# ChanghyeonKim93/nonlinear_optimizer_for_slam

Hardware: AMD Instinct MI355X
Metric: ndt6_gauss_newton_residual_blocks_per_sec (higher is better)
Workload: dtype f64

## Files before the change

nonlinear_optimizer_for_slam_amd/csrc/assemble_one_launch.hpp:

```cpp
#pragma once

#include "assemble_pass.hpp"

namespace nos {

constexpr size_t kSingleBlockMaxElements = size_t(1024) * 15;

template <typename Problem, typename T, int BLOCK, bool NT>
__device__ __forceinline__ int single_block_loop(const TiledLayout& L, typename Problem::Params& P, uint32_t n_chunks,
                                                 LmDevice& s_lm, double* s_sum, double* __restrict__ cost_history,
                                                 int history_capacity) {
  constexpr int kF = Problem::kFields;
  constexpr int kOut = Problem::kOut;
  const T* __restrict__ base = static_cast<const T*>(L.base);
  int executed = 0;
  while (s_lm.st.done == 0) {
    set_pose(P, &s_lm);
    T acc[kOut];
#pragma unroll
    for (int k = 0; k < kOut; ++k) acc[k] = T(0);
    constexpr uint32_t kRound = (kF * sizeof(T) > 64) ? 2 : 4;
    for (uint32_t c = 0; c < n_chunks; c += kRound) {
      T x[kRound][kF][1];
      uint64_t i0[kRound];
// ... 73 lines not shown
      asm volatile("s_waitcnt vmcnt(0)" ::: "memory");
      __hip_atomic_store(seq_host, seq, __ATOMIC_RELAXED, __HIP_MEMORY_SCOPE_SYSTEM);
    }
  }
}

constexpr uint32_t kClusterMaxBlocks = 256;
constexpr unsigned long long kClusterTimeoutTicks = 5000000ull;
constexpr unsigned long long kClusterMailboxTimeoutTicks = kMailboxTimeoutTicks;

struct ClusterCtl {
  unsigned int abort;
  unsigned int pad0[31];
  struct alignas(128) Arrival {
    unsigned int count;
    unsigned int pad[31];
  } arrival[8];
};

__device__ __forceinline__ double sc1_load(const double* p) {
  return __hip_atomic_load(p, __ATOMIC_RELAXED, __HIP_MEMORY_SCOPE_AGENT);
}
__device__ __forceinline__ void sc1_store(double* p, double v) {
  __hip_atomic_store(p, v, __ATOMIC_RELAXED, __HIP_MEMORY_SCOPE_AGENT);
}

__device__ __forceinline__ void state_store_sc1(LmDevice* lm, const nos_host::LmState& st) {
  double* d = reinterpret_cast<double*>(&lm->st);
  const double* s = reinterpret_cast<const double*>(&st);
  constexpr int kWords = int(sizeof(nos_host::LmState) / sizeof(double));
  static_assert(sizeof(nos_host::LmState) % sizeof(double) == 0, "LmState must be a whole number of doubles");
#pragma unroll
  for (int k = 0; k < kWords; ++k) sc1_store(d + k, s[k]);
}
__device__ __forceinline__ void state_load_sc1(const LmDevice* lm, nos_host::LmState& st) {
  const double* d = reinterpret_cast<const double*>(&lm->st);
  double* s = reinterpret_cast<double*>(&st);
  constexpr int kWords = int(sizeof(nos_host::LmState) / sizeof(double));
#pragma unroll
  for (int k = 0; k < kWords; ++k) s[k] = sc1_load(d + k);
}

template <int FIELDS, int ELEM>
struct ResidentShape;
template <>
struct ResidentShape<15, 8> { static constexpr int RI = 3, LI = 3; };
template <>
struct ResidentShape<15, 4> { static constexpr int RI = 3, LI = 4; };
template <>
struct ResidentShape<5, 8> { static constexpr int RI = 9, LI = 7; };
template <>
struct ResidentShape<5, 4> { static constexpr int RI = 10, LI = 14; };

template <typename Problem, typename T, int BLOCK, int RI, int LI, int SI = 0, bool SPF = false, bool NT = false>
__global__ __launch_bounds__(BLOCK) void solve_cluster_kernel(TiledLayout L, typename Problem::Params P,
                                                             double* __restrict__ partials, LmDevice* lm, ClusterCtl* ctl,
                                                             double* __restrict__ cost_history, int history_capacity,
                                                             double* entry_host, unsigned long long* seq_host,
                                                             unsigned long long seq, uint32_t items_per_lane,
                                                             const Mailbox* mail = nullptr, uint32_t stream_lds = 0u) {
  constexpr int kF = Problem::kFields;
  constexpr int kOut = Problem::kOut;
  constexpr int kCols = 32;
  constexpr int kSlices = BLOCK / kCols;
  const T* __restrict__ base = static_cast<const T*>(L.base);
  constexpr int kRF = kF;
  extern __shared__ __align__(16) unsigned char resident_raw[];
  T* resident = reinterpret_cast<T*>(resident_raw);
  __shared__ int s_flag;
  __shared__ int s_fast;
  __shared__ double red[kSlices][kCols];
  __shared__ double s_tot[kLmTotDoubles(kOut)];
  __shared__ double s_lmd_raw[(sizeof(LmDevice) + 7) / 8];
  LmDevice& s_lmd = *reinterpret_cast<LmDevice*>(s_lmd_raw);
  nos_host::LmState& s_state = s_lmd.st;
  [[maybe_unused]] __shared__ double s_local[kCols];
  [[maybe_unused]] __shared__ unsigned long long s_round0;
  const bool multi = mail != nullptr;

  const uint32_t J = items_per_lane & 0x7fffffffu;
  [[maybe_unused]] const bool allow_fast = (items_per_lane >> 31) == 0u;
  [[maybe_unused]] constexpr int kXccCol = 28;
  [[maybe_unused]] const unsigned int my_xcc = xcc_id();
  const uint64_t block_base = uint64_t(blockIdx.x) * BLOCK * J;
  auto fetch = [&](uint32_t j, T (&dst)[kRF]) -> bool {
    const uint64_t i = block_base + uint64_t(j) * BLOCK + threadIdx.x;
    const bool ok = i < L.n;
    const uint64_t ic = ok ? i : 0;
    const uint64_t off = (ic >> L.tile_shift) * L.tile_stride + (ic & L.tile_mask);
    T xt[kF][1];
#pragma unroll
    for (int f = 0; f < kF; ++f) load_items<T, 1, false>(base + field_offset<Problem>(L, ic, off, f), xt[f]);
#pragma unroll
    for (int f = 0; f < kF; ++f) dst[f] = ok ? xt[f][0] : T(0);
    return ok;
  };
  auto evaluate_resident = [&](const T (&xi)[kRF], bool ok, T (&acc_)[kOut]) { Problem::item(xi, P, ok, acc_); };
  T x[RI > 0 ? RI : 1][kRF];
  bool valid[RI > 0 ? RI : 1];
  static_assert(SI == 0 || (RI == 0 && LI == 0), "the streaming form keeps nothing resident");
  constexpr int kSI = SI > 0 ? SI : 1;
  [[maybe_unused]] T xs[kF][kSI];
  [[maybe_unused]] uint64_t xs_i0 = 0;
  [[maybe_unused]] const uint32_t my_rounds = blockIdx.x < J ? (J - blockIdx.x + gridDim.x - 1) / gridDim.x : 0u;
  [[maybe_unused]] const uint32_t lds_k = SI > 0 ? min(stream_lds, my_rounds > 0u ? my_rounds - 1u : 0u) : 0u;
  [[maybe_unused]] const uint32_t lds_r0 = lds_k > 0u ? my_rounds / (lds_k + 1u) : ~0u;
  [[maybe_unused]] const uint32_t lds_r1 = lds_k > 1u ? uint32_t(2ull * my_rounds / (lds_k + 1u)) : ~0u;
  [[maybe_unused]] const uint32_t lds_r2 = lds_k > 2u ? uint32_t(3ull * my_rounds / (lds_k + 1u)) : ~0u;
  [[maybe_unused]] auto lds_round = [&](uint32_t s) -> uint32_t { return s == 0u ? lds_r0 : s == 1u ? lds_r1 : s == 2u ? lds_r2 : ~0u; };
  [[maybe_unused]] auto fetch_chunk = [&](uint32_t c, T (&dst)[kF][kSI]) -> uint64_t {
    const uint64_t i0 = uint64_t(c) * (uint64_t(BLOCK) * kSI) + uint64_t(threadIdx.x) * kSI;
    const uint64_t off = (i0 >> L.tile_shift) * L.tile_stride + (i0 & L.tile_mask);
#pragma unroll
    for (int f = 0; f < kF; ++f) load_items<T, kSI, NT>(base + field_offset<Problem>(L, i0, off, f), dst[f]);
    return i0;
  };
  if constexpr (SI > 0) {
    if (blockIdx.x < J) xs_i0 = fetch_chunk(blockIdx.x, xs);
  }
#pragma unroll
  for (int j = 0; j < RI; ++j) {
    valid[j] = false;
    if (uint32_t(j) < J) {
      valid[j] = fetch(uint32_t(j), x[j]);
    } else {
#pragma unroll
      for (int f = 0; f < kRF; ++f) x[j][f] = T(0);
    }
  }
  if constexpr (LI > 0) {
    for (uint32_t j = RI; j < J; ++j) {
      T xi[kRF];
      (void)fetch(j, xi);
#pragma unroll
      for (int f = 0; f < kRF; ++f) resident[(size_t(j - RI) * kRF + f) * BLOCK + threadIdx.x] = xi[f];
    }
  }
  NOS_PROBE(if (threadIdx.x < 4) s_step_cycles[threadIdx.x] = 0ull;)
  if (threadIdx.x == 0) {
    s_lmd.settings = lm->settings;
    s_state = lm->st;
    s_flag = s_state.done != 0 ? 1 : 0;
    s_fast = 0;
    if (__hip_atomic_load(&ctl->abort, __ATOMIC_RELAXED, __HIP_MEMORY_SCOPE_AGENT) != 0u) s_flag = 2;
    if (multi && blockIdx.x == 0) s_round0 = *mail->round;
  }
  __syncthreads();
  [[maybe_unused]] const unsigned int group = blockIdx.x & 7u;
  const unsigned int n_groups = gridDim.x < 8u ? gridDim.x : 8u;
  unsigned int it = 0;
  int executed = 0;
  NOS_PROBE(unsigned long long tq[6] = {0, 0, 0, 0, 0, 0}, tp = 0;)
#define NOS_RES_STAMP(slot_) NOS_PROBE({ const unsigned long long now_ = wall_clock64(); tq[slot_] += now_ - tp; tp = now_; })
  while (s_flag == 0) {
    NOS_PROBE(tp = wall_clock64();)
    if constexpr (kOut == 28) {
#pragma unroll
      for (int k = 0; k < 9; ++k) P.R[k] = T(uniform_load(&s_state.R[k]));
#pragma unroll
      for (int k = 0; k < 3; ++k) P.t[k] = T(uniform_load(&s_state.t[k]));
    } else {
#pragma unroll
      for (int k = 0; k < 4; ++k) P.R2[k] = T(uniform_load(&s_state.R[k]));
#pragma unroll
      for (int k = 0; k < 2; ++k) P.t2[k] = T(uniform_load(&s_state.t[k]));
    }
    T acc[kOut];
#pragma unroll
    for (int k = 0; k < kOut; ++k) acc[k] = T(0);
    if constexpr (SI > 0) {
      const uint32_t n_chunks = J;
      auto evaluate = [&](const T (&xc)[kF][SI > 0 ? SI : 1], uint64_t i0) {
#pragma unroll
        for (int it = 0; it < (SI > 0 ? SI : 1); ++it) {
          T xi[kF];
#pragma unroll
          for (int f = 0; f < kF; ++f) xi[f] = xc[f][it];
          Problem::item(xi, P, (i0 + it) < L.n, acc);
        }
      };
      if constexpr (SPF) {
        for (uint32_t c = blockIdx.x; c < n_chunks; c += gridDim.x) {
          T xb[kF][SI > 0 ? SI : 1];
          uint64_t i1 = 0;
          const uint32_t cn = c + gridDim.x;
          if (cn < n_chunks) i1 = fetch_chunk(cn, xb);
          evaluate(xs, xs_i0);
#pragma unroll
          for (int f = 0; f < kF; ++f)
#pragma unroll
            for (int it = 0; it < (SI > 0 ? SI : 1); ++it) xs[f][it] = xb[f][it];
          xs_i0 = i1;
        }
      } else {
        auto lds_at = [&](uint32_t s, int f, int e) -> T& {
          return resident[((size_t(s) * kF + f) * BLOCK + threadIdx.x) * kSI + e];
        };
        auto evaluate_lds = [&](uint32_t s, uint32_t cl) {
          const uint64_t i0 = uint64_t(cl) * (uint64_t(BLOCK) * kSI) + uint64_t(threadIdx.x) * kSI;
#pragma unroll
          for (int e = 0; e < kSI; ++e) {
            T xi[kF];
#pragma unroll
            for (int f = 0; f < kF; ++f) xi[f] = lds_at(s, f, e);
            Problem::item(xi, P, (i0 + e) < L.n, acc);
          }
        };
        const bool from_lds = it != 0u;
        uint32_t s = 0;
        uint32_t next_res = lds_round(0u);
        auto evaluate_lds_rounds = [&](uint32_t k0, uint32_t k1) {
          for (uint32_t kr = k0; kr < k1; ++kr) {
            evaluate_lds(s, blockIdx.x + kr * gridDim.x);
            next_res = lds_round(++s);
          }
        };
        for (uint32_t k = 0; k < my_rounds;) {
          __builtin_amdgcn_sched_barrier(0);
          if (!from_lds && k == next_res) {
#pragma unroll
            for (int f = 0; f < kF; ++f)
#pragma unroll
              for (int e = 0; e < kSI; ++e) lds_at(s, f, e) = xs[f][e];
            next_res = lds_round(++s);
          }
          evaluate(xs, xs_i0);
          uint32_t kn = k + 1u;
          if (from_lds)
            for (uint32_t sn = s; kn == lds_round(sn); ++sn) ++kn;
          xs_i0 = fetch_chunk(blockIdx.x + (kn < my_rounds ? kn : 0u) * gridDim.x, xs);
          evaluate_lds_rounds(k + 1u, kn);
          k = kn;
        }
      }
      if constexpr (SPF) {
        if (blockIdx.x < n_chunks) xs_i0 = fetch_chunk(blockIdx.x, xs);
      }
    } else
    if (sizeof(T) == 8 && J >= uint32_t(RI)) {
#pragma unroll
      for (int j = 0; j < RI; ++j) evaluate_resident(x[j], valid[j], acc);
    } else {
#pragma unroll
      for (int j = 0; j < RI; ++j)
        if (uint32_t(j) < J) evaluate_resident(x[j], valid[j], acc);
    }
    if constexpr (LI > 0) {
      for (uint32_t j = RI; j < J; ++j) {
        T xi[kRF];
#pragma unroll
        for (int f = 0; f < kRF; ++f) xi[f] = resident[(size_t(j - RI) * kRF + f) * BLOCK + threadIdx.x];
        evaluate_resident(xi, (block_base + uint64_t(j) * BLOCK + threadIdx.x) < L.n, acc);
      }
    }
    double dacc[kOut];
#pragma unroll
    for (int k = 0; k < kOut; ++k) dacc[k] = double(acc[k]);
    NOS_RES_STAMP(0)
    {
      TaggedUnit* const block_units = reinterpret_cast<TaggedUnit*>(partials);
      TaggedUnit* const group_units = block_units + size_t(kClusterMaxBlocks) * 32;
      const unsigned long long tag = (seq << 24) | ((unsigned long long)it + 1ull);
      const double mine = block_reduce_value<kOut, BLOCK>(dacc);
      const bool probe = it == 0u && allow_fast;
      if (threadIdx.x < kOut) {
        if (s_fast != 0)
          tagged_store_plain(block_units + size_t(blockIdx.x) * 32 + threadIdx.x, mine, tag);
        else
          tagged_store(block_units + size_t(blockIdx.x) * 32 + threadIdx.x, mine, tag);
      } else if (probe && threadIdx.x == kXccCol) {
        tagged_store(block_units + size_t(blockIdx.x) * 32 + kXccCol, double(my_xcc), tag);
      }
      NOS_RES_STAMP(1)
      const unsigned long long deadline = wall_clock64() + (multi ? kClusterMailboxTimeoutTicks : kClusterTimeoutTicks);
      auto await = [&](const TaggedUnit* u, double* value) -> bool {
        unsigned int polls = 0;
        for (;;) {
          const TaggedUnit got = tagged_load(u);
          if (got.seq == tag) {
            *value = got.value;
            return true;
          }
          if ((++polls & 63u) == 0u &&
              (__hip_atomic_load(&ctl->abort, __ATOMIC_RELAXED, __HIP_MEMORY_SCOPE_AGENT) != 0u || wall_clock64() > deadline)) {
            __hip_atomic_store(&ctl->abort, 1u, __ATOMIC_RELAXED, __HIP_MEMORY_SCOPE_AGENT);
// ... 204 lines not shown
```

nonlinear_optimizer_for_slam_amd/csrc/nos_core.hip:

```cpp
#include "nos_internal.hpp"
#if defined(__x86_64__) && !defined(__HIP_DEVICE_COMPILE__)
#include <emmintrin.h>
#endif

#include <cxxabi.h>

namespace nosd {

namespace {
thread_local std::string g_last_error;
}

int fail(int status, const char* fmt, ...) {
  char buf[512];
  va_list ap;
  va_start(ap, fmt);
  vsnprintf(buf, sizeof buf, fmt, ap);
  va_end(ap);
  g_last_error = buf;
  return status;
}

const char* last_error_text() { return g_last_error.c_str(); }
void clear_last_error() { g_last_error.clear(); }
// ... 142 lines not shown
  constexpr bool kReproj = Problem::kFields == 5;
  if constexpr (sizeof(T) == 8) {
    if (variant == 0 && kReproj) variant = 7;
    switch (variant) {
      NOS_CASE(0, 1, 512, 3, 1)
      NOS_CASE(1, 1, 256, 3, 2)
      NOS_CASE(3, 2, 256, 2, 2)
      NOS_CASE_PP(7, 1, 512, kReproj ? 3 : 2, 1)
#ifdef NOS_ALL_VARIANTS
      NOS_CASE(2, 1, 256, 2, 2)
      NOS_CASE(4, 2, 512, 2, 1)
      NOS_CASE_PP(8, 2, 512, 2, 1)
#endif
    }
  } else {
    if (variant == 0) variant = kReproj ? 11 : 1;
    switch (variant) {
      NOS_CASE(1, 2, 512, 2, 1)
      NOS_CASE_PP(11, 2, 512, 2, 1)
#ifdef NOS_ALL_VARIANTS
      NOS_CASE(2, 1, 256, 4, 2)
      NOS_CASE(3, 2, 256, 5, 2)
      NOS_CASE(4, 2, 256, 4, 2)
      NOS_CASE(5, 1, 1024, 4, 1)
      NOS_CASE(6, 2, 1024, 4, 1)
      NOS_CASE(9, 2, 256, 3, 3)
      NOS_CASE_PP(12, 4, 512, 2, 1)
      NOS_CASE(13, 4, 256, 2, 1)
#endif
    }
  }
#undef NOS_CASE
#undef NOS_CASE_PP
  return fail(NOS_ERR_UNSUPPORTED, "launch geometry %d is not compiled into this build for this element type "
              "(default build: fp64 0, 1, 3, 7; fp32 1, 11; `make ALL_VARIANTS=1` builds the rest)", variant);
}

size_t resident_items_per_lane(int n_fields, int dtype) {
  if (n_fields == 15)
    return dtype == NOS_F64 ? size_t(nos::ResidentShape<15, 8>::RI + nos::ResidentShape<15, 8>::LI)
                            : size_t(nos::ResidentShape<15, 4>::RI + nos::ResidentShape<15, 4>::LI);
  if (n_fields == 5)
    return dtype == NOS_F64 ? size_t(nos::ResidentShape<5, 8>::RI + nos::ResidentShape<5, 8>::LI)
                            : size_t(nos::ResidentShape<5, 4>::RI + nos::ResidentShape<5, 4>::LI);
  return 1;
}

struct SingleBlockArgs {
  int cluster_blocks = 0;
  int items_per_lane = 1;
  int stream_chunks = 0;
  bool nt = false;
  int stream_lds_chunks = 0;
  bool stage1_sc1 = false;
  const nos::Mailbox* mail = nullptr;
  double* partials = nullptr;
  nos::ClusterCtl* ctl = nullptr;
  nos::LmDevice* lm;
  double* history;
  int history_capacity;
  double* entry;
  unsigned long long* seq_host;
  unsigned long long seq;
};

template <typename Problem, typename T>
int launch_single(const nos::TiledLayout& L, const typename Problem::Params& P, const SingleBlockArgs& a, hipStream_t stream) {
  constexpr int kBlock = 512;
  if (L.n_padded % kBlock != 0) return fail(NOS_ERR_INVALID_ARGUMENT, "n_padded %% 512 != 0");
  if (a.cluster_blocks > 0 && a.stream_chunks > 0) {
    constexpr int kSI = sizeof(T) == 8 ? 1 : 2;
    constexpr bool kSPF = false;
    constexpr size_t kChunk = size_t(kBlock) * kSI;
    if (L.n_padded % kChunk != 0 || (L.tile_stride != 0 && ((size_t(L.tile_mask) + 1) % kChunk) != 0))
      return fail(NOS_ERR_INVALID_ARGUMENT, "streaming solve: layout not a multiple of the %zu-item chunk", kChunk);
    if (size_t(a.stream_chunks) * kChunk != L.n_padded) return fail(NOS_ERR_INVALID_ARGUMENT, "streaming solve: chunk count does not match the layout");
    const auto kernel = a.nt ? nos::solve_cluster_kernel<Problem, T, kBlock, 0, 0, kSI, kSPF, true>
                             : nos::solve_cluster_kernel<Problem, T, kBlock, 0, 0, kSI, kSPF, false>;
    uint32_t lds = uint32_t(std::min(std::max(a.stream_lds_chunks, 0), 3));
    size_t dyn_bytes = lds * size_t(Problem::kFields) * kChunk * sizeof(T);
    if (dyn_bytes > size_t(48) * 1024 &&
        hipFuncSetAttribute(reinterpret_cast<const void*>(kernel), hipFuncAttributeMaxDynamicSharedMemorySize,
                            int(dyn_bytes)) != hipSuccess) {
      (void)hipGetLastError();
      lds = 0;
      dyn_bytes = 0;
    }
    t_last_kernel = reinterpret_cast<const void*>(kernel);
    hipLaunchKernelGGL(kernel, dim3(a.cluster_blocks), dim3(kBlock), dyn_bytes, stream, L, P, a.partials, a.lm, a.ctl, a.history,
                       a.history_capacity, a.entry, a.seq_host, a.seq, uint32_t(a.stream_chunks) | (a.stage1_sc1 ? 0x80000000u : 0u),
                       a.mail, lds);
    hipError_t e = hipGetLastError();
    if (e != hipSuccess) return fail(NOS_ERR_HIP, "streaming solve launch failed: %s", hipGetErrorString(e));
    return NOS_OK;
  }
  if (a.cluster_blocks > 0) {
    using Shape = nos::ResidentShape<Problem::kPlanes, int(sizeof(T))>;
    if (a.items_per_lane < 1 || a.items_per_lane > Shape::RI + Shape::LI)
      return fail(NOS_ERR_INVALID_ARGUMENT, "resident solve: %d items per lane do not fit (%d + %d)", a.items_per_lane,
                  Shape::RI, Shape::LI);
    const auto kernel = nos::solve_cluster_kernel<Problem, T, kBlock, Shape::RI, Shape::LI>;
    const size_t lds_items = a.items_per_lane > Shape::RI ? size_t(a.items_per_lane - Shape::RI) : 0;
    const size_t dyn_bytes = lds_items * size_t(Problem::kFields) * kBlock * sizeof(T);
    if (dyn_bytes > size_t(48) * 1024) {
      const hipError_t ea = hipFuncSetAttribute(reinterpret_cast<const void*>(kernel),
                                                hipFuncAttributeMaxDynamicSharedMemorySize, int(dyn_bytes));
      if (ea != hipSuccess) return fail(NOS_ERR_UNSUPPORTED, "resident solve: %zu bytes of LDS refused: %s", dyn_bytes, hipGetErrorString(ea));
    }
    t_last_kernel = reinterpret_cast<const void*>(kernel);
    hipLaunchKernelGGL(kernel, dim3(a.cluster_blocks), dim3(kBlock), dyn_bytes, stream, L, P, a.partials, a.lm, a.ctl,
                       a.history, a.history_capacity, a.entry, a.seq_host, a.seq,
                       uint32_t(a.items_per_lane) | (a.stage1_sc1 ? 0x80000000u : 0u), a.mail, 0u);
    hipError_t e = hipGetLastError();
    if (e != hipSuccess) return fail(NOS_ERR_HIP, "cluster solve launch failed: %s", hipGetErrorString(e));
    return NOS_OK;
  }
  const uint32_t n_chunks = uint32_t((std::max<uint64_t>(L.n, 1) + kBlock - 1) / kBlock);
  t_last_kernel = reinterpret_cast<const void*>(&nos::solve_single_block_kernel<Problem, T, kBlock>);
  hipLaunchKernelGGL((nos::solve_single_block_kernel<Problem, T, kBlock>), dim3(1), dim3(kBlock), 0, stream, L, P, n_chunks, a.lm,
                     a.history, a.history_capacity, a.entry, a.seq_host, a.seq);
  hipError_t e = hipGetLastError();
  if (e != hipSuccess) return fail(NOS_ERR_HIP, "single-workgroup solve launch failed: %s", hipGetErrorString(e));
  return NOS_OK;
}

template <template <typename, int> class ProblemT, typename T, typename ParamsT>
int launch_by_loss(int loss_kind, int variant, int blocks_per_cu, int num_cus,
                   const nos::TiledLayout& L, const ParamsT& P, bool nt, double* partials,
                   const nos::FusedFinal& fin, hipStream_t stream, int* rows_out, const SingleBlockArgs* single = nullptr) {
  switch (loss_kind) {
    case NOS_LOSS_NONE:
      if (single) return launch_single<ProblemT<T, nos::kLossNone>, T>(L, P, *single, stream);
      return launch_by_variant<ProblemT<T, nos::kLossNone>, T>(variant, blocks_per_cu, num_cus, L, P, nt, partials,
                                                               fin, stream, rows_out);
    case NOS_LOSS_EXPONENTIAL:
      if (single) return launch_single<ProblemT<T, nos::kLossExponential>, T>(L, P, *single, stream);
      return launch_by_variant<ProblemT<T, nos::kLossExponential>, T>(variant, blocks_per_cu, num_cus, L, P, nt,
                                                                      partials, fin, stream, rows_out);
    case NOS_LOSS_HUBER:
      if (single) return launch_single<ProblemT<T, nos::kLossHuber>, T>(L, P, *single, stream);
      return launch_by_variant<ProblemT<T, nos::kLossHuber>, T>(variant, blocks_per_cu, num_cus, L, P, nt, partials,
                                                                fin, stream, rows_out);
  }
  return fail(NOS_ERR_INVALID_ARGUMENT, "unknown loss kind %d", loss_kind);
}

int check_loss(const nos_loss* loss, int* kind_out) {
  int kind = loss ? loss->kind : NOS_LOSS_NONE;
  if (kind < NOS_LOSS_NONE || kind > NOS_LOSS_HUBER) return fail(NOS_ERR_INVALID_ARGUMENT, "unknown loss kind %d", kind);
  if (kind == NOS_LOSS_EXPONENTIAL && (loss->a < 0.0 || loss->b < 0.0))
    return fail(NOS_ERR_INVALID_ARGUMENT, "exponential loss needs c1 >= 0 and c2 >= 0");
  if (kind == NOS_LOSS_HUBER && !(loss->a > 0.0)) return fail(NOS_ERR_INVALID_ARGUMENT, "huber loss needs threshold > 0");
  *kind_out = kind;
  return NOS_OK;
}

bool use_nontemporal(const nos_dataset* ds, const Shard& sh) {
  const int force = ds->ctx->settings.nt;
  if (force >= 0) return force != 0;
  return sh.bytes > (size_t(192) << 20);
}

int launch_assemble_raw(const nos_dataset* ds, const Shard& sh, const Request& rq, double* partials,
                        const nos::FusedFinal& fin, hipStream_t stream, int* rows_out,
                        const SingleBlockArgs* single = nullptr);
// ... 361 lines not shown
    st.done = int(e[nos::kLogDone]);
    st.ok = int(e[nos::kLogOk]);
    const int executed = int(e[nos::kLogExecuted]);
    if (slot.prof_on && slot.prof_every == 0) slot.prof_launches += executed;
    if (opt->cost_history != nullptr)
      for (int k = 0; k < executed && k < opt->max_iterations; ++k) opt->cost_history[k] = slot.h_hist[k];
    for (int k = 0; k < nR; ++k) R[k] = st.R[k];
    for (int k = 0; k < nt; ++k) t[k] = st.t[k];
    if (report) {
      report->iterations = st.iteration;
      report->ok = st.ok;
      report->launches = 1;
      report->fallback = 0;
      report->printed_cost = st.previous_cost;
      report->last_cost = st.cost;
      report->final_lambda = st.lambda;
    }
    return NOS_OK;
  }
  const size_t max_blocks = std::min<size_t>(std::min<size_t>(nos::kClusterMaxBlocks, size_t(slot.num_cus)),
                                             size_t(std::max(1, ctx->settings.lm_cluster_max_blocks)));
  const bool mailbox_in_launch = ctx->shm_dev != nullptr && ctx->d_peers != nullptr && ctx->d_mail != nullptr &&
                                 ds->kind != kKindNdtIndexed;
  int fell_back = 0;
  const size_t cluster_blocks = std::min<size_t>(max_blocks, (sh.layout.n + 511) / 512);
  const size_t items_per_lane = cluster_blocks > 0 ? (sh.layout.n + cluster_blocks * 512 - 1) / (cluster_blocks * 512) : 0;
  const size_t resident_capacity = ctx->settings.lm_cluster == 2 ? 1 : resident_items_per_lane(ds->n_fields, ds->dtype);
  const size_t stream_chunk = size_t(512) * (ds->dtype == NOS_F64 ? 1 : 2);
  const bool resident_fits = items_per_lane >= 1 && items_per_lane <= resident_capacity;
  const bool stream_form = !resident_fits && (ctx->settings.lm_cluster == 1 || ctx->settings.lm_cluster == 5) && items_per_lane >= 1 &&
                           sh.layout.n_padded % stream_chunk == 0 && sh.layout.n_padded / stream_chunk < (size_t(1) << 31) &&
                           (sh.layout.tile_stride == 0 || (size_t(sh.layout.tile_mask) + 1) % stream_chunk == 0);
  bool paused = false;
  if (mailbox_in_launch) {
    paused = slot.cluster_paused_solves > 0;
    if (paused) --slot.cluster_paused_solves;
  } else {
    if (slot.cluster_gave_up &&
        std::chrono::steady_clock::now() - slot.cluster_gave_up_at > std::chrono::milliseconds(ctx->settings.lm_cluster_retry_ms))
      slot.cluster_gave_up = false;
    paused = slot.cluster_gave_up;
  }
  if (ds->kind != kKindNdtIndexed && !with_comm && (ctx->shm_dev == nullptr || mailbox_in_launch) && opt->max_iterations > 0 &&
      cluster_blocks >= 1 && (resident_fits || stream_form) && !paused &&
      ctx->settings.lm_cluster != 0 && (opt->cost_history == nullptr || opt->max_iterations <= kHistCapacity)) {
    SingleBlockArgs cl{};
    cl.cluster_blocks = int(cluster_blocks);
    cl.items_per_lane = int(items_per_lane);
    if (stream_form) {
      cl.items_per_lane = 0;
      cl.stream_chunks = int(sh.layout.n_padded / stream_chunk);
      cl.nt = use_nontemporal(ds, sh);
      cl.stream_lds_chunks = ctx->settings.stream_lds_chunks;
    }
    cl.stage1_sc1 = ctx->settings.lm_cluster == 5;
    cl.mail = mailbox_in_launch ? ctx->d_mail : nullptr;
    cl.partials = slot.partials;
    cl.ctl = slot.d_cluster;
    cl.lm = slot.d_lm;
    cl.history = opt->cost_history ? slot.h_hist_dev : nullptr;
    cl.history_capacity = kHistCapacity;
    cl.entry = slot.h_log_dev;
    cl.seq_host = seq_dev;
    cl.seq = ++slot.seq;
    NOS_HIP_CHECK(hipMemsetAsync(slot.d_cluster, 0, sizeof(nos::ClusterCtl), slot.stream));
    if (ctx->settings.debug_cluster_abort != 0) {
      const unsigned int raised = 1u;
      NOS_HIP_CHECK(hipMemcpyAsync(&slot.d_cluster->abort, &raised, sizeof raised, hipMemcpyHostToDevice, slot.stream));
      NOS_HIP_CHECK(hipStreamSynchronize(slot.stream));
    }
    int rows = 0;
    const int rc_launch = launch_assemble_raw(ds, sh, rq, slot.partials, nos::FusedFinal{}, slot.stream, &rows, &cl);
    if (rc_launch != NOS_OK && rc_launch != NOS_ERR_UNSUPPORTED) return rc_launch;
    const bool launched_ok = rc_launch == NOS_OK;
    volatile unsigned long long* seqw = reinterpret_cast<volatile unsigned long long*>(slot.h_out + kSeqSlot);
    bool finished = false;
    for (long spins = 0; launched_ok && spins < 4000000; ++spins) {
      if (*seqw >= cl.seq) {
        finished = true;
        break;
      }
#if defined(__x86_64__)
      __builtin_ia32_pause();
#endif
    }
    if (!finished) {
      NOS_HIP_CHECK(hipStreamSynchronize(slot.stream));
      finished = *seqw >= cl.seq;
    }
    if (finished) {
      __atomic_thread_fence(__ATOMIC_ACQUIRE);
      slot.cluster_next_pause = 64;
      const double* e = slot.h_log;
      for (int k = 0; k < 9; ++k) st.R[k] = e[nos::kLogR + k];
      for (int k = 0; k < 3; ++k) st.t[k] = e[nos::kLogT + k];
      st.lambda = e[nos::kLogLambda];
      st.previous_cost = e[nos::kLogPrevCost];
      st.cost = e[nos::kLogCost];
      st.iteration = int(e[nos::kLogIteration]);
      st.done = int(e[nos::kLogDone]);
      st.ok = int(e[nos::kLogOk]);
      const int executed = int(e[nos::kLogExecuted]);
#ifdef NOS_LM_TIMING
      fprintf(stderr, "[resident-timing] %d blocks x %d items/lane (0 = streamed), %d iterations; workgroup 0, us per iteration: item math %.2f, "
              "block reduce %.2f, drain+arrive+wait %.2f, rows->sums %.2f, LM step+barrier %.2f\n", cl.cluster_blocks,
              cl.items_per_lane, executed, e[50] * 0.01, e[51] * 0.01, e[52] * 0.01, e[53] * 0.01, e[54] * 0.01);
// ... 589 lines not shown
}


int zero_pad(int dtype, int n_fields, const nos::TiledLayout& L, void* dst, hipStream_t stream) {
  return dtype == NOS_F64 ? zero_pad_launch<double>(n_fields, L, dst, stream) : zero_pad_launch<float>(n_fields, L, dst, stream);
}

int unpack_records(int dtype, const unsigned char* d_rec, size_t stride, const nos::FieldOffsets& fo, int n_fields,
                   size_t first, size_t count, const nos::TiledLayout& L, void* dst, hipStream_t stream) {
  return dtype == NOS_F64 ? unpack_launch<double>(d_rec, stride, fo, n_fields, first, count, L, dst, stream)
                          : unpack_launch<float>(d_rec, stride, fo, n_fields, first, count, L, dst, stream);
}

}

using namespace nosd;


extern "C" {

namespace {
void drop_out_of_range_settings(nosd::Settings& st);
}

int nos_ctx_create(const int* device_ids, int n_devices, nos_ctx** out_ctx) {
  if (!out_ctx) return fail(NOS_ERR_INVALID_ARGUMENT, "out_ctx is NULL");
  *out_ctx = nullptr;
  if (n_devices < 1 || n_devices > 64 || !device_ids) return fail(NOS_ERR_INVALID_ARGUMENT, "bad device list");
  int count = 0;
  hipError_t e = hipGetDeviceCount(&count);
  if (e != hipSuccess || count < 1)
    return fail(NOS_ERR_NO_DEVICE, "no usable HIP device (%s); this library has no CPU fallback",
                e != hipSuccess ? hipGetErrorString(e) : "device count is 0");
  for (int i = 0; i < n_devices; ++i)
    if (device_ids[i] < 0 || device_ids[i] >= count)
      return fail(NOS_ERR_INVALID_ARGUMENT, "device id %d out of range [0,%d)", device_ids[i], count);
  nos_ctx* ctx = new (std::nothrow) nos_ctx();
  if (!ctx) return fail(NOS_ERR_OUT_OF_MEMORY, "host allocation failed");
  ctx->slots.resize(n_devices);
  ctx->blocks_per_cu = env_int("NOS_BLOCKS_PER_CU", 0);
  ctx->variant = env_int("NOS_VARIANT", 0);
  {
    Settings& st = ctx->settings;
    st.plane_skew = env_int("NOS_PLANE_SKEW", st.plane_skew);
    st.sc1 = env_int("NOS_SC1", st.sc1);
    st.nt = env_int("NOS_NT", st.nt);
    st.fused = env_int("NOS_FUSED", st.fused);
    st.lm_fused = env_int("NOS_LM_FUSED", st.lm_fused);
    st.lm_window = env_int("NOS_LM_WINDOW", st.lm_window);
    st.lm_single = env_int("NOS_LM_SINGLE", st.lm_single);
    st.lm_cluster = env_int("NOS_LM_CLUSTER", st.lm_cluster);
    st.lm_cluster_max_blocks = env_int("NOS_LM_CLUSTER_MAX_BLOCKS", st.lm_cluster_max_blocks);
    st.stream_lds_chunks = env_int("NOS_STREAM_LDS_CHUNKS", st.stream_lds_chunks);
    st.batch_max_elements = env_int("NOS_BATCH_MAX_ELEMENTS", st.batch_max_elements);
    st.pool = env_int("NOS_POOL", st.pool);
    st.tile_log2 = env_int("NOS_TILE_LOG2", int(kDefaultTileLog2));
    const char* ingest = getenv("NOS_INGEST");
    st.ingest = (ingest && !strcmp(ingest, "pack")) ? 1 : ((ingest && !strcmp(ingest, "unpack")) ? 2 : 0);
    st.ingest_threads = env_int("NOS_INGEST_THREADS", 0);
    st.indexed_bpc = env_int("NOS_INDEXED_BPC", st.indexed_bpc);
    st.match_dense = env_int("NOS_MATCH_DENSE", st.match_dense);
    st.map_compact_keys = env_int("NOS_MAP_COMPACT_KEYS", st.map_compact_keys);
    st.pgo_host_scalars = env_int("NOS_PGO_HOST_SCALARS", st.pgo_host_scalars);
    st.pgo_precond = env_int("NOS_PGO_PRECOND", st.pgo_precond);
    st.pgo_agg = env_int("NOS_PGO_AGG", st.pgo_agg);
    st.pgo_block = env_int("NOS_PGO_BLOCK", st.pgo_block);
    st.pgo_coarse_probe = env_int("NOS_PGO_COARSE_PROBE", st.pgo_coarse_probe);
    drop_out_of_range_settings(st);
  }
  for (int i = 0; i < n_devices; ++i) {
    DeviceSlot& s = ctx->slots[i];
    s.device = device_ids[i];
    s.pool_enabled = ctx->settings.pool != 0;
    hipDeviceProp_t prop;
    e = hipSetDevice(s.device);
    if (e == hipSuccess) e = hipGetDeviceProperties(&prop, s.device);
    if (e == hipSuccess) {
      s.num_cus = prop.multiProcessorCount > 0 ? prop.multiProcessorCount : 256;
      e = hipStreamCreateWithFlags(&s.own_stream, hipStreamNonBlocking);
    }
    if (e == hipSuccess) e = hipMalloc(&s.partials, sizeof(double) * kMaxPartialRows * kMaxOut);
    if (e == hipSuccess) e = hipMalloc(&s.d_out, sizeof(double) * kMaxOut);
    if (e == hipSuccess) e = hipHostMalloc(&s.h_out, sizeof(double) * 64, hipHostMallocMapped);
    if (e == hipSuccess) memset(s.h_out, 0, sizeof(double) * 64);
    if (e == hipSuccess) e = hipHostGetDevicePointer(reinterpret_cast<void**>(&s.h_out_dev), s.h_out, 0);
    if (e == hipSuccess) e = hipMalloc(&s.d_lm, sizeof(nos::LmDevice));
    const size_t log_bytes = sizeof(double) * kLogSlots * nos::kLogEntryDoubles;
    if (e == hipSuccess) e = hipHostMalloc(&s.h_log, log_bytes, hipHostMallocMapped);
    if (e == hipSuccess) memset(s.h_log, 0, log_bytes);
    if (e == hipSuccess) e = hipHostGetDevicePointer(reinterpret_cast<void**>(&s.h_log_dev), s.h_log, 0);
    if (e == hipSuccess) e = hipMalloc(reinterpret_cast<void**>(&s.d_cluster), sizeof(nos::ClusterCtl));
    if (e == hipSuccess) e = hipMemset(s.d_cluster, 0, sizeof(nos::ClusterCtl));
    if (e == hipSuccess) e = hipHostMalloc(&s.h_hist, sizeof(double) * kHistCapacity, hipHostMallocMapped);
    if (e == hipSuccess) e = hipHostGetDevicePointer(reinterpret_cast<void**>(&s.h_hist_dev), s.h_hist, 0);
    if (e == hipSuccess) e = hipMalloc(&s.counter, 2048);
    if (e == hipSuccess) e = hipMemset(s.counter, 0, 2048);
    if (e == hipSuccess) e = hipEventCreate(&s.ev0);
    if (e == hipSuccess) e = hipEventCreate(&s.ev1);
    if (e == hipSuccess) e = hipEventCreate(&s.ev2);
    s.stream = s.own_stream;
    if (e != hipSuccess) {
      nos_ctx_destroy(ctx);
      return fail(e == hipErrorOutOfMemory ? NOS_ERR_OUT_OF_MEMORY : NOS_ERR_HIP, "context setup failed on device %d: %s",
                  device_ids[i], hipGetErrorString(e));
    }
  }
// ... 84 lines not shown

int nos_ctx_num_devices(const nos_ctx* ctx) { return ctx ? int(ctx->slots.size()) : 0; }

int nos_ctx_set_stream(nos_ctx* ctx, int shard, void* hip_stream) {
  nosd::CtxGuard guard_(ctx);
  if (!ctx || shard < 0 || shard >= int(ctx->slots.size())) return fail(NOS_ERR_INVALID_ARGUMENT, "bad ctx / shard");
  ctx->slots[shard].stream = hip_stream ? static_cast<hipStream_t>(hip_stream) : ctx->slots[shard].own_stream;
  return NOS_OK;
}

int nos_ctx_synchronize(nos_ctx* ctx) {
  nosd::CtxGuard guard_(ctx);
  if (!ctx) return fail(NOS_ERR_INVALID_ARGUMENT, "ctx is NULL");
  for (DeviceSlot& s : ctx->slots) {
    NOS_HIP_CHECK(hipSetDevice(s.device));
    NOS_HIP_CHECK(hipStreamSynchronize(s.stream));
  }
  return NOS_OK;
}

namespace {
struct OptionEntry {
  const char* key;
  int nosd::Settings::*field;
  int lo, hi;
};
const OptionEntry kOptions[] = {
    {"plane_skew", &nosd::Settings::plane_skew, 0, 1 << 20},
    {"sc1", &nosd::Settings::sc1, 0, 1},
    {"nt", &nosd::Settings::nt, -1, 1},
    {"fused", &nosd::Settings::fused, 0, 1},
    {"lm_fused", &nosd::Settings::lm_fused, 0, 1},
    {"lm_window", &nosd::Settings::lm_window, 1, nosd::kLogSlots - 2},
    {"lm_single", &nosd::Settings::lm_single, 0, 1},
    {"lm_cluster", &nosd::Settings::lm_cluster, 0, 5},
    {"lm_cluster_retry_ms", &nosd::Settings::lm_cluster_retry_ms, 0, 3600000},
    {"pool", &nosd::Settings::pool, 0, 1},
    {"tile_log2", &nosd::Settings::tile_log2, -1, 24},
    {"ingest", &nosd::Settings::ingest, 0, 2},
    {"ingest_threads", &nosd::Settings::ingest_threads, 0, 1024},
    {"indexed_bpc", &nosd::Settings::indexed_bpc, 1, 16},
    {"match_dense", &nosd::Settings::match_dense, 0, 1},
    {"map_compact_keys", &nosd::Settings::map_compact_keys, 0, 1},
    {"pgo_host_scalars", &nosd::Settings::pgo_host_scalars, 0, 1},
    {"pgo_precond", &nosd::Settings::pgo_precond, 0, 1},
    {"pgo_agg", &nosd::Settings::pgo_agg, 2, 1 << 20},
    {"pgo_block", &nosd::Settings::pgo_block, 0, 1},
    {"pgo_coarse_probe", &nosd::Settings::pgo_coarse_probe, 0, 1},
    {"map_fma_mask", &nosd::Settings::map_fma_mask, 0, (1 << 26) - 1},
    {"map_eigen_version", &nosd::Settings::map_eigen_version, 33, 34},
    {"debug_cluster_abort", &nosd::Settings::debug_cluster_abort, 0, 2},
    {"lm_cluster_max_blocks", &nosd::Settings::lm_cluster_max_blocks, 1, 256},
    {"stream_lds_chunks", &nosd::Settings::stream_lds_chunks, 0, 3},
    {"batch_max_elements", &nosd::Settings::batch_max_elements, 0, 1 << 30},
};
bool option_in_range(const OptionEntry& o, int value);
void drop_out_of_range_settings(nosd::Settings& st) {
  const nosd::Settings defaults;
  for (const OptionEntry& o : kOptions)
    if (!option_in_range(o, st.*(o.field))) {
      fprintf(stderr, "[nos-hip] NOS_%s = %d is outside [%d, %d]: ignored\n", o.key, st.*(o.field), o.lo, o.hi);
      st.*(o.field) = defaults.*(o.field);
    }
}
bool option_in_range(const OptionEntry& o, int value) {
  if (value < o.lo || value > o.hi) return false;
  if (!strcmp(o.key, "tile_log2")) return value <= 0 || value >= 10;
  return true;
}
}

int nos_ctx_set_option(nos_ctx* ctx, const char* key, int value) {
  if (!ctx || !key) return fail(NOS_ERR_INVALID_ARGUMENT, "ctx / key is NULL");
  nosd::CtxGuard guard_(ctx);
  for (const OptionEntry& o : kOptions)
    if (!strcmp(o.key, key)) {
      if (!option_in_range(o, value))
        return fail(NOS_ERR_INVALID_ARGUMENT, "option '%s' = %d is outside [%d, %d]", key, value, o.lo, o.hi);
      ctx->settings.*(o.field) = value;
      for (DeviceSlot& s : ctx->slots) s.pool_enabled = ctx->settings.pool != 0;
      return NOS_OK;
    }
  return fail(NOS_ERR_INVALID_ARGUMENT, "unknown option '%s'", key);
}

int nos_ctx_get_option(const nos_ctx* ctx, const char* key, int* value) {
  if (!ctx || !key || !value) return fail(NOS_ERR_INVALID_ARGUMENT, "ctx / key / value is NULL");
  nosd::CtxGuard guard_(ctx);
  for (const OptionEntry& o : kOptions)
    if (!strcmp(o.key, key)) {
      *value = ctx->settings.*(o.field);
      return NOS_OK;
    }
  return fail(NOS_ERR_INVALID_ARGUMENT, "unknown option '%s'", key);
}

int nos_runtime_info(char* buf, size_t capacity) {
  if (!buf || capacity == 0) return fail(NOS_ERR_INVALID_ARGUMENT, "buf is NULL");
  int runtime = 0, driver = 0;
  (void)hipRuntimeGetVersion(&runtime);
  (void)hipDriverGetVersion(&driver);
  std::string hip_file;
  const std::string hip_dir = dir_of_symbol(reinterpret_cast<const void*>(&hipGetDeviceCount), &hip_file);
  RcclApi* api = Rccl();
  int rccl_version = 0;
  if (api->ok && api->GetVersion) (void)api->GetVersion(&rccl_version);
// ... 617 lines not shown
```

nonlinear_optimizer_for_slam_amd/csrc/nos_internal.hpp:

```cpp
#pragma once

#include <hip/hip_runtime.h>
#include <dlfcn.h>
#include <fcntl.h>
#include <sys/mman.h>
#include <sys/stat.h>
#include <unistd.h>
#include <rccl/rccl.h>

#include <algorithm>
#include <atomic>
#include <chrono>
#include <random>
#include <climits>
#include <cmath>
#include <cstdarg>
#include <cstdio>
#include <cstdlib>
#include <cstring>
#include <map>
#include <memory>
#include <new>
#include <string>
#include <thread>
// ... 74 lines not shown
  size_t batch_pinned_bytes = 0;
  hipEvent_t pack_done[2] = {nullptr, nullptr};
  struct PoolEntry {
    void* ptr;
    size_t bytes;
  };
  std::vector<PoolEntry> pool;
  size_t pool_bytes = 0;
  bool pool_enabled = true;
  const void* last_kernel = nullptr;
  bool cluster_gave_up = false;
  std::chrono::steady_clock::time_point cluster_gave_up_at{};
  int cluster_paused_solves = 0;
  int cluster_next_pause = 64;
  std::vector<hipEvent_t> prof_events;
  size_t prof_used = 0;
  bool prof_on = false;
  int prof_every = 1;
  long prof_launches = 0;
};


}

namespace nosd {
constexpr int kMapReferenceFmaMask = (4 | 8 | 16 | 32) | ((1 | 4 | 8 | 32 | 256) << 8) | (0x1ff << 17);
struct Settings {
  int plane_skew = 1088;
  int sc1 = 1;
  int nt = -1;
  int fused = 1;
  int lm_fused = 1;
  int lm_window = 3;
  int lm_single = 1;
  int lm_cluster_retry_ms = 5000;
  int lm_cluster = 1;
  int pool = 1;
  int tile_log2 = -1;
  int ingest = 0;
  int ingest_threads = 0;
  int indexed_bpc = 1;
  int match_dense = 1;
  int map_compact_keys = 1;
  int pgo_host_scalars = 0;
  int pgo_precond = 1;
  int pgo_agg = 48;
  int pgo_coarse_probe = 0;
  int pgo_block = 1;
  int map_fma_mask = kMapReferenceFmaMask;
  int map_eigen_version = 34;
  int debug_cluster_abort = 0;
  int lm_cluster_max_blocks = 256;
  int stream_lds_chunks = 3;
  int batch_max_elements = int(nos::kSingleBlockMaxElements);
};
}

struct nos_ctx {
  std::recursive_mutex mu;
  nosd::Settings settings;
  std::vector<nosd::DeviceSlot> slots;
  int blocks_per_cu = 0;
  int variant = 0;
  int tile_log2 = -1;
  ncclComm_t comm = nullptr;
  int comm_ranks = 1;
  int comm_rank = 0;
  void* shm_host = nullptr;
  size_t shm_bytes = 0;
  double* shm_dev = nullptr;
  unsigned long long* d_round = nullptr;
  nos::Mailbox* d_mail = nullptr;
  double* ipc_own = nullptr;
  std::vector<double*> ipc_peers;
  double** d_peers = nullptr;
};

namespace nosd {

struct CtxGuard {
  std::unique_lock<std::recursive_mutex> lock;
  explicit CtxGuard(const nos_ctx* ctx) {
    if (ctx != nullptr) lock = std::unique_lock<std::recursive_mutex>(const_cast<nos_ctx*>(ctx)->mu);
  }
};

struct Shard {
  int slot = 0;
  nos::TiledLayout layout{};
  void* data = nullptr;
  size_t bytes = 0;
  size_t capacity = 0;
  bool pooled = false;
  int32_t* index = nullptr;
  void* table = nullptr;
  bool one_block = false;
  int n_slots = 0;
  size_t n_voxels = 0;
};

}

struct nos_dataset {
  nos_ctx* ctx = nullptr;
  int kind = 0;
  int dtype = NOS_F64;
// ... 147 lines not shown
```

Measured before the change: 75.38 billion.

## Keep extra streamed chunks resident in registers across LM iterations

```diff
diff --git a/nonlinear_optimizer_for_slam_amd/csrc/assemble_one_launch.hpp b/nonlinear_optimizer_for_slam_amd/csrc/assemble_one_launch.hpp
--- a/nonlinear_optimizer_for_slam_amd/csrc/assemble_one_launch.hpp
+++ b/nonlinear_optimizer_for_slam_amd/csrc/assemble_one_launch.hpp
@@ -149,13 +149,20 @@
 template <>
 struct ResidentShape<5, 4> { static constexpr int RI = 10, LI = 14; };
 
+template <typename Problem, typename T>
+struct StreamRegRounds { static constexpr int kRR = 3; };
+template <int LOSS>
+struct StreamRegRounds<Ndt6Problem<float, LOSS>, float> { static constexpr int kRR = 0; };
+constexpr int kStreamRegRoundsMax = 3;
+
 template <typename Problem, typename T, int BLOCK, int RI, int LI, int SI = 0, bool SPF = false, bool NT = false>
 __global__ __launch_bounds__(BLOCK) void solve_cluster_kernel(TiledLayout L, typename Problem::Params P,
                                                              double* __restrict__ partials, LmDevice* lm, ClusterCtl* ctl,
                                                              double* __restrict__ cost_history, int history_capacity,
                                                              double* entry_host, unsigned long long* seq_host,
                                                              unsigned long long seq, uint32_t items_per_lane,
-                                                             const Mailbox* mail = nullptr, uint32_t stream_lds = 0u) {
+                                                             const Mailbox* mail = nullptr, uint32_t stream_lds = 0u,
+                                                             uint32_t stream_reg = 0u) {
   constexpr int kF = Problem::kFields;
   constexpr int kOut = Problem::kOut;
   constexpr int kCols = 32;
@@ -199,11 +206,32 @@
   constexpr int kSI = SI > 0 ? SI : 1;
   [[maybe_unused]] T xs[kF][kSI];
   [[maybe_unused]] uint64_t xs_i0 = 0;
+  [[maybe_unused]] constexpr int kRR = (SI > 0 && !SPF) ? StreamRegRounds<Problem, T>::kRR : 0;
+  static_assert(kRR <= kStreamRegRoundsMax, "the option's range covers every instantiation");
+  [[maybe_unused]] T xr[kRR > 0 ? kRR : 1][kF][kSI];
   [[maybe_unused]] const uint32_t my_rounds = blockIdx.x < J ? (J - blockIdx.x + gridDim.x - 1) / gridDim.x : 0u;
   [[maybe_unused]] const uint32_t lds_k = SI > 0 ? min(stream_lds, my_rounds > 0u ? my_rounds - 1u : 0u) : 0u;
-  [[maybe_unused]] const uint32_t lds_r0 = lds_k > 0u ? my_rounds / (lds_k + 1u) : ~0u;
-  [[maybe_unused]] const uint32_t lds_r1 = lds_k > 1u ? uint32_t(2ull * my_rounds / (lds_k + 1u)) : ~0u;
-  [[maybe_unused]] const uint32_t lds_r2 = lds_k > 2u ? uint32_t(3ull * my_rounds / (lds_k + 1u)) : ~0u;
+  [[maybe_unused]] const uint32_t reg_k = kRR > 0 ? min(min(stream_reg, uint32_t(kRR)), (my_rounds > 0u ? my_rounds - 1u : 0u) - lds_k) : 0u;
+  [[maybe_unused]] const uint32_t alt_k = min(lds_k, reg_k);
+  [[maybe_unused]] auto chip_round = [&](uint32_t i) -> uint32_t {
+    return uint32_t(uint64_t(i + 1u) * my_rounds / (lds_k + reg_k + 1u));
+  };
+  [[maybe_unused]] auto lds_slot_round = [&](uint32_t sl) -> uint32_t {
+    return sl < lds_k ? chip_round(sl < alt_k ? 2u * sl : alt_k + sl) : ~0u;
+  };
+  [[maybe_unused]] const uint32_t lds_r0 = lds_slot_round(0u);
+  [[maybe_unused]] const uint32_t lds_r1 = lds_slot_round(1u);
+  [[maybe_unused]] const uint32_t lds_r2 = lds_slot_round(2u);
+  [[maybe_unused]] uint32_t reg_r[kRR > 0 ? kRR : 1];
+#pragma unroll
+  for (int j = 0; j < (kRR > 0 ? kRR : 1); ++j)
+    reg_r[j] = uint32_t(j) < reg_k ? chip_round(uint32_t(j) < alt_k ? 2u * uint32_t(j) + 1u : alt_k + uint32_t(j)) : ~0u;
+#pragma unroll
+  for (int j = 0; j < (kRR > 0 ? kRR : 1); ++j)
+#pragma unroll
+    for (int f = 0; f < kF; ++f)
+#pragma unroll
+      for (int e = 0; e < kSI; ++e) xr[j][f][e] = T(0);
   [[maybe_unused]] auto lds_round = [&](uint32_t s) -> uint32_t { return s == 0u ? lds_r0 : s == 1u ? lds_r1 : s == 2u ? lds_r2 : ~0u; };
   [[maybe_unused]] auto fetch_chunk = [&](uint32_t c, T (&dst)[kF][kSI]) -> uint64_t {
     const uint64_t i0 = uint64_t(c) * (uint64_t(BLOCK) * kSI) + uint64_t(threadIdx.x) * kSI;
@@ -303,31 +331,91 @@
             Problem::item(xi, P, (i0 + e) < L.n, acc);
           }
         };
-        const bool from_lds = it != 0u;
+        const bool on_chip = it != 0u;
         uint32_t s = 0;
         uint32_t next_res = lds_round(0u);
-        auto evaluate_lds_rounds = [&](uint32_t k0, uint32_t k1) {
-          for (uint32_t kr = k0; kr < k1; ++kr) {
-            evaluate_lds(s, blockIdx.x + kr * gridDim.x);
-            next_res = lds_round(++s);
-          }
+        auto in_registers = [&](uint32_t r) -> bool {
+          bool hit = false;
+#pragma unroll
+          for (int j = 0; j < kRR; ++j) hit = hit || r == reg_r[j];
+          return hit;
         };
-        for (uint32_t k = 0; k < my_rounds;) {
-          __builtin_amdgcn_sched_barrier(0);
-          if (!from_lds && k == next_res) {
-#pragma unroll
-            for (int f = 0; f < kF; ++f)
-#pragma unroll
-              for (int e = 0; e < kSI; ++e) lds_at(s, f, e) = xs[f][e];
-            next_res = lds_round(++s);
-          }
-          evaluate(xs, xs_i0);
-          uint32_t kn = k + 1u;
-          if (from_lds)
-            for (uint32_t sn = s; kn == lds_round(sn); ++sn) ++kn;
-          xs_i0 = fetch_chunk(blockIdx.x + (kn < my_rounds ? kn : 0u) * gridDim.x, xs);
-          evaluate_lds_rounds(k + 1u, kn);
-          k = kn;
+        uint32_t k = 0;
+        if constexpr (kRR == 0) {
+          while (k < my_rounds) {
+            __builtin_amdgcn_sched_barrier(0);
+            if (!on_chip && k == next_res) {
+#pragma unroll
+              for (int f = 0; f < kF; ++f)
+#pragma unroll
+                for (int e = 0; e < kSI; ++e) lds_at(s, f, e) = xs[f][e];
+              next_res = lds_round(++s);
+            }
+            evaluate(xs, xs_i0);
+            uint32_t kn = k + 1u;
+            if (on_chip)
+              for (uint32_t sn = s; kn == lds_round(sn); ++sn) ++kn;
+            xs_i0 = fetch_chunk(blockIdx.x + (kn < my_rounds ? kn : 0u) * gridDim.x, xs);
+            for (uint32_t kr = k + 1u; kr < kn; ++kr) {
+              evaluate_lds(s, blockIdx.x + kr * gridDim.x);
+              next_res = lds_round(++s);
+            }
+            k = kn;
+          }
+        } else
+#pragma unroll
+        for (int j = 0; j <= kRR; ++j) {
+          const uint32_t rj = j < kRR ? reg_r[j < kRR ? j : 0] : ~0u;
+          const uint32_t stop = min(rj, my_rounds);
+          const uint32_t hi = (!on_chip && rj != ~0u) ? rj + 1u : stop;
+          auto lds_rounds_below = [&](uint32_t lim) {
+            while (next_res < lim) {
+              evaluate_lds(s, blockIdx.x + next_res * gridDim.x);
+              next_res = lds_round(++s);
+            }
+          };
+          if (on_chip && j > 0) lds_rounds_below(min(k, stop));
+          while (k < hi) {
+            __builtin_amdgcn_sched_barrier(0);
+            if (!on_chip) {
+              if (k == next_res) {
+#pragma unroll
+                for (int f = 0; f < kF; ++f)
+#pragma unroll
+                  for (int e = 0; e < kSI; ++e) lds_at(s, f, e) = xs[f][e];
+                next_res = lds_round(++s);
+              }
+              if constexpr (kRR > 0) {
+                if (j < kRR && k == rj) {
+#pragma unroll
+                  for (int f = 0; f < kF; ++f)
+#pragma unroll
+                    for (int e = 0; e < kSI; ++e) xr[j < kRR ? j : 0][f][e] = xs[f][e];
+                }
+              }
+            }
+            evaluate(xs, xs_i0);
+            uint32_t kn = k + 1u;
+            if (on_chip) {
+              for (uint32_t sn = s;;) {
+                if (kn == lds_round(sn)) {
+                  ++sn;
+                  ++kn;
+                } else if (in_registers(kn)) {
+                  ++kn;
+                } else {
+                  break;
+                }
+              }
+            }
+            xs_i0 = fetch_chunk(blockIdx.x + (kn < my_rounds ? kn : 0u) * gridDim.x, xs);
+            if (on_chip) lds_rounds_below(min(kn, stop));
+            k = kn;
+          }
+          if constexpr (kRR > 0) {
+            if (j < kRR && on_chip && rj != ~0u)
+              evaluate(xr[j < kRR ? j : 0], uint64_t(blockIdx.x + rj * gridDim.x) * (uint64_t(BLOCK) * kSI) + uint64_t(threadIdx.x) * kSI);
+          }
         }
       }
       if constexpr (SPF) {
diff --git a/nonlinear_optimizer_for_slam_amd/csrc/nos_core.hip b/nonlinear_optimizer_for_slam_amd/csrc/nos_core.hip
--- a/nonlinear_optimizer_for_slam_amd/csrc/nos_core.hip
+++ b/nonlinear_optimizer_for_slam_amd/csrc/nos_core.hip
@@ -218,6 +218,7 @@
   int stream_chunks = 0;
   bool nt = false;
   int stream_lds_chunks = 0;
+  int stream_reg_rounds = 0;
   bool stage1_sc1 = false;
   const nos::Mailbox* mail = nullptr;
   double* partials = nullptr;
@@ -252,10 +253,11 @@
       lds = 0;
       dyn_bytes = 0;
     }
+    const uint32_t reg = uint32_t(std::min(std::max(a.stream_reg_rounds, 0), nos::kStreamRegRoundsMax));
     t_last_kernel = reinterpret_cast<const void*>(kernel);
     hipLaunchKernelGGL(kernel, dim3(a.cluster_blocks), dim3(kBlock), dyn_bytes, stream, L, P, a.partials, a.lm, a.ctl, a.history,
                        a.history_capacity, a.entry, a.seq_host, a.seq, uint32_t(a.stream_chunks) | (a.stage1_sc1 ? 0x80000000u : 0u),
-                       a.mail, lds);
+                       a.mail, lds, reg);
     hipError_t e = hipGetLastError();
     if (e != hipSuccess) return fail(NOS_ERR_HIP, "streaming solve launch failed: %s", hipGetErrorString(e));
     return NOS_OK;
@@ -276,7 +278,7 @@
     t_last_kernel = reinterpret_cast<const void*>(kernel);
     hipLaunchKernelGGL(kernel, dim3(a.cluster_blocks), dim3(kBlock), dyn_bytes, stream, L, P, a.partials, a.lm, a.ctl,
                        a.history, a.history_capacity, a.entry, a.seq_host, a.seq,
-                       uint32_t(a.items_per_lane) | (a.stage1_sc1 ? 0x80000000u : 0u), a.mail, 0u);
+                       uint32_t(a.items_per_lane) | (a.stage1_sc1 ? 0x80000000u : 0u), a.mail, 0u, 0u);
     hipError_t e = hipGetLastError();
     if (e != hipSuccess) return fail(NOS_ERR_HIP, "cluster solve launch failed: %s", hipGetErrorString(e));
     return NOS_OK;
@@ -744,6 +746,7 @@
       cl.stream_chunks = int(sh.layout.n_padded / stream_chunk);
       cl.nt = use_nontemporal(ds, sh);
       cl.stream_lds_chunks = ctx->settings.stream_lds_chunks;
+      cl.stream_reg_rounds = ctx->settings.stream_reg_rounds;
     }
     cl.stage1_sc1 = ctx->settings.lm_cluster == 5;
     cl.mail = mailbox_in_launch ? ctx->d_mail : nullptr;
@@ -1439,6 +1442,7 @@
     st.lm_cluster = env_int("NOS_LM_CLUSTER", st.lm_cluster);
     st.lm_cluster_max_blocks = env_int("NOS_LM_CLUSTER_MAX_BLOCKS", st.lm_cluster_max_blocks);
     st.stream_lds_chunks = env_int("NOS_STREAM_LDS_CHUNKS", st.stream_lds_chunks);
+    st.stream_reg_rounds = env_int("NOS_STREAM_REG_ROUNDS", st.stream_reg_rounds);
     st.batch_max_elements = env_int("NOS_BATCH_MAX_ELEMENTS", st.batch_max_elements);
     st.pool = env_int("NOS_POOL", st.pool);
     st.tile_log2 = env_int("NOS_TILE_LOG2", int(kDefaultTileLog2));
@@ -1629,6 +1633,7 @@
     {"debug_cluster_abort", &nosd::Settings::debug_cluster_abort, 0, 2},
     {"lm_cluster_max_blocks", &nosd::Settings::lm_cluster_max_blocks, 1, 256},
     {"stream_lds_chunks", &nosd::Settings::stream_lds_chunks, 0, 3},
+    {"stream_reg_rounds", &nosd::Settings::stream_reg_rounds, 0, nos::kStreamRegRoundsMax},
     {"batch_max_elements", &nosd::Settings::batch_max_elements, 0, 1 << 30},
 };
 bool option_in_range(const OptionEntry& o, int value);
diff --git a/nonlinear_optimizer_for_slam_amd/csrc/nos_internal.hpp b/nonlinear_optimizer_for_slam_amd/csrc/nos_internal.hpp
--- a/nonlinear_optimizer_for_slam_amd/csrc/nos_internal.hpp
+++ b/nonlinear_optimizer_for_slam_amd/csrc/nos_internal.hpp
@@ -150,6 +150,7 @@
   int debug_cluster_abort = 0;
   int lm_cluster_max_blocks = 256;
   int stream_lds_chunks = 3;
+  int stream_reg_rounds = 3;
   int batch_max_elements = int(nos::kSingleBlockMaxElements);
 };
 }
```

New measurement: 77.41 billion, median of 6. 1.03x the previous value.
